# zprodev/zlib.es

Measured on AMD Instinct MI355X. Metric: GiB/s deflate+inflate round trip, 64 MiB buffers (uncompressed bytes / wall), bit-exact vs reference, higher is better.
Workload: dtype u8; 1 GPU; random64: 1 x 64 MiB xorshift buffer(s) per GPU (seed 12345+index), deflate then inflate, HBM-resident; bytes_per_buffer=67108864, compressed_bytes=67176156, parallelism=independent buffers, one per GPU

## Files before the change

zlib.es_amd/csrc/zes_deflate.hip:

```cpp
#include "zes_common.h"
#include "zes_kernels.h"

__device__ static inline uint32_t lds_ld32u(const uint8_t* s, uint32_t off) {
  const uint32_t* w = reinterpret_cast<const uint32_t*>(s);
  uint32_t i = off >> 2;
  uint32_t lo = w[i], hi = w[i + 1];
  return __builtin_amdgcn_alignbyte(hi, lo, off & 3u);
}

__device__ static inline void stage_block(uint8_t* s, const uint8_t* g, uint32_t bytes, uint32_t padded) {
  const uint32_t tid = threadIdx.x, nth = blockDim.x;
  const uint32_t mis = (uint32_t)((uintptr_t)g & 15u);
  if (mis == 0) {
    const uint4* g4 = reinterpret_cast<const uint4*>(g);
    uint4* s4 = reinterpret_cast<uint4*>(s);
    const uint32_t full = bytes >> 4;
    for (uint32_t i = tid; i < full; i += nth) s4[i] = g4[i];
    for (uint32_t i = (full << 4) + tid; i < padded; i += nth) s[i] = i < bytes ? g[i] : (uint8_t)0;
  } else {
    for (uint32_t i = tid; i < padded; i += nth) s[i] = i < bytes ? g[i] : (uint8_t)0;
  }
}

__device__ unsigned long long* g_sort_dbg = nullptr;
// ... 2191 lines not shown
      if ((int)lane >= d) incl += t;
    }
    if (lane == 63) S.wsum[wave] = incl;
    __syncthreads();
    uint32_t base = 14u + 3u * HCLEN, total = 0;
    for (uint32_t w = 0; w < HUFF_THREADS / 64; w++) {
      if (w < wave) base += S.wsum[w];
      total += S.wsum[w];
    }
    uint32_t bp = base + incl - mine;
    if (tb[0]) hdr_or(S, bp, tv[0], tb[0]);
    bp += tb[0];
    if (tb[1]) hdr_or(S, bp, tv[1], tb[1]);
    if (tid == 0) S.hdr_bits = 14u + 3u * HCLEN + total;
  }
  __syncthreads();
  USTAMP(6);
  uint32_t part = 0;
  for (uint32_t s = tid; s < 286; s += HUFF_THREADS) {
    uint32_t xb = (s >= 257) ? kLenXbits[s - 257] : 0u;
    part += hg[s] * ((uint32_t)S.lens[s] + xb);
  }
  if (tid < 30) part += hg[288 + tid] * ((uint32_t)S.lens[288 + tid] + kDistXbits[tid]);
  atomicAdd(&S.total_bits, part);
  __syncthreads();
  if (tid == 0) {
    blks[g].hdr_bits = S.hdr_bits;
    blks[g].bits = 3u + S.hdr_bits + S.total_bits;
  }
  uint32_t* cg = codes_out + (uint64_t)g * 320;
  for (uint32_t i = tid; i < 320; i += HUFF_THREADS) cg[i] = (uint32_t)S.codes[i] | ((uint32_t)S.lens[i] << 16);
  uint32_t* hd = hdr_out + (uint64_t)g * ZES_HDR_WORDS;
  for (uint32_t i = tid; i < ZES_HDR_WORDS; i += HUFF_THREADS) hd[i] = S.hdr[i];
  USTAMP(7);
}

__global__ __launch_bounds__(HUFF_THREADS) void k_huff_lengths_only(const uint32_t* __restrict__ hist, uint32_t nsym, uint32_t L,
                                                                    uint8_t* __restrict__ lens_out) {
  __shared__ HuffSmem S;
  const uint32_t tid = threadIdx.x;
  for (uint32_t i = tid; i < 320; i += HUFF_THREADS) S.hist[i] = i < nsym ? hist[i] : 0u;
  __syncthreads();
  pm_lengths(S, S.hist, nsym, L, S.lens);
  for (uint32_t i = tid; i < nsym; i += HUFF_THREADS) lens_out[i] = S.lens[i];
}

__global__ void k_make_blks(ZesBuf b0, uint32_t nbuf, ZesBuf* __restrict__ bufs, ZesBlk* __restrict__ blks, uint32_t nblk,
                            unsigned long long* __restrict__ adler) {
  const uint32_t i = blockIdx.x * blockDim.x + threadIdx.x;
  if (nbuf == 1u && i == 0) bufs[0] = b0;
  if (i < 2u * nbuf) adler[i] = 0ull;
  if (i >= nblk) return;
  uint32_t lo = 0, hi = nbuf;
  while (hi - lo > 1) {
    const uint32_t mid = (lo + hi) >> 1;
    if ((nbuf == 1u ? b0.first_blk : bufs[mid].first_blk) <= i) lo = mid; else hi = mid;
  }
  const uint64_t n = nbuf == 1u ? b0.n : bufs[lo].n;
  const uint32_t fb = nbuf == 1u ? b0.first_blk : bufs[lo].first_blk;
  ZesBlk z;
  z.buf = lo;
  z.blk = i - fb;
  z.len = (uint32_t)min((uint64_t)ZES_BLK, n - (uint64_t)z.blk * ZES_BLK);
  z.ntok = 0;
  z.hdr_bits = 0;
  z.bits = 0;
  z.bit_off = 0;
  blks[i] = z;
}

__device__ __forceinline__ static void adler_group_sums(uint4 v, uint32_t& a, uint32_t& w) {
  a = __builtin_amdgcn_udot4(v.x, 0x01010101u, 0u, false);
  a = __builtin_amdgcn_udot4(v.y, 0x01010101u, a, false);
  a = __builtin_amdgcn_udot4(v.z, 0x01010101u, a, false);
  a = __builtin_amdgcn_udot4(v.w, 0x01010101u, a, false);
  w = __builtin_amdgcn_udot4(v.x, 0x0D0E0F10u, 0u, false);
  w = __builtin_amdgcn_udot4(v.y, 0x090A0B0Cu, w, false);
  w = __builtin_amdgcn_udot4(v.z, 0x05060708u, w, false);
  w = __builtin_amdgcn_udot4(v.w, 0x01020304u, w, false);
}

__device__ __forceinline__ static void adler_chunk(const uint8_t* __restrict__ p0, uint64_t n, uint64_t c0, uint64_t clen,
                                                   unsigned long long* __restrict__ acc) {
  __shared__ uint64_t sa[ADLER_THREADS / 64], sb[ADLER_THREADS / 64];
  const uint32_t tid = threadIdx.x, lane = tid & 63u, wave = tid >> 6;
  const uint8_t* p = p0 + c0;
  uint64_t A = 0, B = 0;
  const bool aligned = (((uintptr_t)p) & 15u) == 0;
  uint64_t o_first = (uint64_t)tid * 16;
  if (aligned) {
    constexpr uint64_t ROUND = (uint64_t)ADLER_THREADS * 16 * 4;
    const uint64_t nround = clen / ROUND;
    for (uint64_t r = 0; r < nround; r++) {
      uint4 v[4];
#pragma unroll
      for (uint32_t q = 0; q < 4; q++) v[q] = *reinterpret_cast<const uint4*>(p + r * ROUND + (uint64_t)q * ADLER_THREADS * 16 + (uint64_t)tid * 16);
#pragma unroll
      for (uint32_t q = 0; q < 4; q++) {
        const uint64_t o = r * ROUND + (uint64_t)q * ADLER_THREADS * 16 + (uint64_t)tid * 16;
        uint32_t a, w;
        adler_group_sums(v[q], a, w);
        A += a;
        B += (uint64_t)w + (uint64_t)a * (clen - o - 16);
      }
    }
    o_first += nround * ROUND;
  }
  for (uint64_t o = o_first; o < clen; o += (uint64_t)ADLER_THREADS * 16) {
    uint8_t b[16];
    if (aligned && o + 16 <= clen) {
      *reinterpret_cast<uint4*>(b) = *reinterpret_cast<const uint4*>(p + o);
    } else {
#pragma unroll
      for (int k = 0; k < 16; k++) b[k] = (o + k < clen) ? p[o + k] : (uint8_t)0;
    }
    uint32_t a = 0, w = 0;
#pragma unroll
    for (int k = 0; k < 16; k++) {
      a += b[k];
      w += (uint32_t)(16 - k) * b[k];
    }
    A += a;
    B += (uint64_t)w + (uint64_t)a * (clen - o - 16);
  }
  for (int d = 32; d >= 1; d >>= 1) {
    A += __shfl_down(A, d);
    B += __shfl_down(B, d);
  }
  if (lane == 0) {
    sa[wave] = A;
    sb[wave] = B;
  }
  __syncthreads();
  if (tid == 0) {
    uint64_t ta = 0, tb = 0;
    for (uint32_t w = 0; w < ADLER_THREADS / 64; w++) {
      ta += sa[w];
      tb += sb[w];
    }
    const uint64_t after = n - c0 - clen;
    ta %= 65521u;
    tb %= 65521u;
    const uint64_t share = (tb + ta * (after % 65521u)) % 65521u;
    atomicAdd(&acc[0], (unsigned long long)ta);
    atomicAdd(&acc[1], (unsigned long long)share);
  }
}

__global__ __launch_bounds__(ADLER_THREADS) void k_adler(const uint8_t* __restrict__ d_in, uint64_t in_off, uint64_t n,
                                                         unsigned long long* __restrict__ acc) {
  const uint64_t c0 = (uint64_t)blockIdx.x * ADLER_CHUNK;
  adler_chunk(d_in + in_off, n, c0, min((uint64_t)ADLER_CHUNK, n - c0), acc);
}

__global__ __launch_bounds__(ADLER_THREADS) void k_adler_blocks(const uint8_t* __restrict__ d_in, const ZesBuf* __restrict__ bufs,
                                                                const ZesBlk* __restrict__ blks,
                                                                unsigned long long* __restrict__ acc) {
  const ZesBlk bk = blks[blockIdx.x];
  const ZesBuf bf = bufs[bk.buf];
  adler_chunk(d_in + bf.in_off, bf.n, (uint64_t)bk.blk * ZES_BLK, bk.len, acc + 2 * (size_t)bk.buf);
}

__device__ __forceinline__ static uint4 adler_low_bytes(uint32_t n) {
  const uint64_t lo = n >= 8u ? ~0ull : (1ull << (8u * n)) - 1ull;
  const uint64_t hi = n <= 8u ? 0ull : (n >= 16u ? ~0ull : (1ull << (8u * (n - 8u))) - 1ull);
  return make_uint4((uint32_t)lo, (uint32_t)(lo >> 32), (uint32_t)hi, (uint32_t)(hi >> 32));
}

__device__ __forceinline__ static void adler_seg_group(uint4 v, uint32_t o, uint32_t keep_lo, uint32_t keep_hi, uint64_t behind, uint64_t& A,
                                                       uint64_t& B) {
  if (o < keep_lo || o + 16u > keep_hi) {
    const uint4 ml = adler_low_bytes(keep_lo > o ? keep_lo - o : 0u);
    const uint4 mh = adler_low_bytes(keep_hi > o ? min(keep_hi - o, 16u) : 0u);
    v.x &= mh.x & ~ml.x;
    v.y &= mh.y & ~ml.y;
    v.z &= mh.z & ~ml.z;
    v.w &= mh.w & ~ml.w;
  }
  uint32_t a, w;
  adler_group_sums(v, a, w);
  A += a;
  B += (uint64_t)w + (uint64_t)a * behind;
}

__global__ __launch_bounds__(ADLER_THREADS) void k_adler_seg(const uint8_t* __restrict__ d_in, const ZesCrcSeg* __restrict__ segs,
                                                             const uint2* __restrict__ work, unsigned long long* __restrict__ acc) {
  __shared__ uint64_t sa[ADLER_THREADS / 64], sb[ADLER_THREADS / 64];
  const uint32_t tid = threadIdx.x, lane = tid & 63u, wave = tid >> 6;
  const uint2 wk = work[blockIdx.x];
  const ZesCrcSeg sg = segs[wk.x];
  const uint64_t a = (uint64_t)(uintptr_t)d_in + sg.off, end = a + sg.len;
  const uint64_t lo = (a & ~15ull) + (uint64_t)wk.y * ADLER_CHUNK;
  const uint64_t hi = min(lo + ADLER_CHUNK, (end + 15ull) & ~15ull);
  const uint32_t span = (uint32_t)(hi - lo);
  const uint32_t keep_lo = a > lo ? (uint32_t)(a - lo) : 0u;
  const uint32_t keep_hi = (uint32_t)(min(end, hi) - lo);
  const uint4* __restrict__ p = reinterpret_cast<const uint4*>((uintptr_t)lo);
  uint64_t A = 0, B = 0;
  constexpr uint32_t ROUND = ADLER_THREADS * 16u * 4u;
  const uint32_t nround = span / ROUND;
  for (uint32_t r = 0; r < nround; r++) {
    uint4 v[4];
#pragma unroll
    for (uint32_t q = 0; q < 4; q++) v[q] = p[(r * ROUND + q * ADLER_THREADS * 16u) / 16u + tid];
#pragma unroll
    for (uint32_t q = 0; q < 4; q++) {
      const uint32_t o = r * ROUND + q * ADLER_THREADS * 16u + tid * 16u;
      adler_seg_group(v[q], o, keep_lo, keep_hi, (uint64_t)keep_hi - o - 16u, A, B);
    }
  }
  for (uint32_t o = nround * ROUND + tid * 16u; o < span; o += ADLER_THREADS * 16u)
    adler_seg_group(p[o / 16u], o, keep_lo, keep_hi, (uint64_t)keep_hi - o - 16u, A, B);
  for (int d = 32; d >= 1; d >>= 1) {
    A += __shfl_down(A, d);
    B += __shfl_down(B, d);
  }
  if (lane == 0) {
    sa[wave] = A;
    sb[wave] = B;
  }
  __syncthreads();
  if (tid == 0) {
    uint64_t ta = 0, tb = 0;
    for (uint32_t w = 0; w < ADLER_THREADS / 64; w++) {
      ta += sa[w];
      tb += sb[w];
    }
    const uint64_t after = end - min(end, hi);
    ta %= 65521u;
    tb %= 65521u;
    const uint64_t share = (tb + ta * (after % 65521u)) % 65521u;
    atomicAdd(&acc[2 * (size_t)wk.x], (unsigned long long)ta);
    atomicAdd(&acc[2 * (size_t)wk.x + 1], (unsigned long long)share);
  }
}

__global__ __launch_bounds__(256) void k_layout(uint8_t* __restrict__ d_out, const ZesBuf* __restrict__ bufs,
                                                ZesBlk* __restrict__ blks, const unsigned long long* __restrict__ adler_acc,
                                                ZesRes* __restrict__ res) {
  __shared__ uint64_t s_tot;
  __shared__ uint64_t s_part[256];
  const uint32_t b = blockIdx.x, tid = threadIdx.x;
  const ZesBuf bf = bufs[b];
  ZesBlk* bk = blks + bf.first_blk;
  uint32_t* out32 = reinterpret_cast<uint32_t*>(d_out + bf.out_off);
  {
    const uint32_t per = (bf.nblk + 255u) / 256u;
    const uint32_t lo = min(bf.nblk, tid * per), hi = min(bf.nblk, lo + per);
    uint64_t sum = 0;
    for (uint32_t i = lo; i < hi; i++) sum += bk[i].bits;
    s_part[tid] = sum;
    __syncthreads();
    if (tid == 0) {
      uint64_t off = (bf.flags & ZES_BUF_RANGE) ? bf.start_bit : 16;
      for (uint32_t t = 0; t < 256; t++) {
        const uint64_t v = s_part[t];
        s_part[t] = off;
        off += v;
      }
      s_tot = off;
    }
    __syncthreads();
    uint64_t off = s_part[tid];
    for (uint32_t i = lo; i < hi; i++) {
      bk[i].bit_off = off;
      off += bk[i].bits;
    }
  }
  __syncthreads();
  const uint64_t tot = s_tot;
  const bool range = (bf.flags & ZES_BUF_RANGE) != 0;
  const uint64_t raw_end = (tot + 7) >> 3;
  const uint64_t out_len = raw_end + (range ? 0 : 4);
  for (uint32_t i = tid; i < bf.nblk; i += 256) {
    const uint64_t s = bk[i].bit_off, e = s + bk[i].bits - 1;
    if (!(i == 0 && (bf.flags & ZES_BUF_CONT) && (s & 31u))) out32[s >> 5] = 0;
    out32[e >> 5] = 0;
  }
  __syncthreads();
  if (tid == 0) {
    const uint64_t last_dw = (tot - 1) >> 5;
    const uint64_t end_dw = (out_len * 8 - 1) >> 5;
    for (uint64_t w = last_dw + 1; w <= end_dw; w++) out32[w] = 0;
    __threadfence();
    const uint64_t n = bf.n;
    const uint32_t s1 = (uint32_t)((1ull + adler_acc[2 * b + 0]) % 65521ull);
    const uint32_t s2 = (uint32_t)((n % 65521ull + adler_acc[2 * b + 1]) % 65521ull);
    const uint32_t ad = (s2 << 16) | s1;
    if (!range) {
      atomicOr(&out32[0], 0x9C78u);
      for (int k = 0; k < 4; k++) {
        const uint64_t pos = raw_end + k;
        const uint32_t byte = (ad >> (24 - 8 * k)) & 0xffu;
        atomicOr(&out32[pos >> 2], byte << (8 * (pos & 3)));
      }
    }
    res[b].out_len = range ? tot - bf.start_bit : out_len;
    res[b].status = 0;
    res[b].aux = ad;
  }
}

#ifndef EMIT_ITEMS
#define EMIT_ITEMS 4
#endif
#define EMIT_TILE (EMIT_THREADS * EMIT_ITEMS)
#define EMIT_STAGE_WORDS (EMIT_TILE * 48 / 32 + 8)
struct EmitSmem {
  uint32_t codes[320];
  uint32_t stage[EMIT_STAGE_WORDS];
  uint32_t wsum[EMIT_THREADS / 64];
  uint32_t carry;
};

__device__ static inline void stage_or(uint32_t* stage, uint32_t rel_bit, uint64_t v, uint32_t nbits) {
  const uint32_t w = rel_bit >> 5, sh = rel_bit & 31u;
  const uint64_t lo = v << sh;
  atomicOr(&stage[w], (uint32_t)lo);
  if (sh + nbits > 32u) atomicOr(&stage[w + 1], (uint32_t)(lo >> 32));
  if (sh + nbits > 64u) atomicOr(&stage[w + 2], (uint32_t)(v >> (64u - sh)));
}

__device__ __forceinline__ static void emit_lds_barrier() { asm volatile("s_waitcnt lgkmcnt(0)\n\ts_barrier" ::: "memory"); }

__global__ __launch_bounds__(EMIT_THREADS, 8) void k_emit(uint8_t* __restrict__ d_out, const ZesBuf* __restrict__ bufs,
                                                       const ZesBlk* __restrict__ blks, const uint32_t* __restrict__ tok_in,
                                                       const uint32_t* __restrict__ codes_in, const uint32_t* __restrict__ hdr_in) {
  __shared__ EmitSmem S;
  const uint32_t g = blockIdx.x, tid = threadIdx.x, lane = tid & 63u, wave = tid >> 6;
  const ZesBlk bk = blks[g];
  const ZesBuf bf = bufs[bk.buf];
  uint32_t* out32 = reinterpret_cast<uint32_t*>(d_out + bf.out_off);
  const uint32_t* tk = tok_in + (uint64_t)g * ZES_BLK;
  const uint32_t* hd = hdr_in + (uint64_t)g * ZES_HDR_WORDS;
  for (uint32_t i = tid; i < 320; i += EMIT_THREADS) S.codes[i] = codes_in[(uint64_t)g * 320 + i];
  if (tid == 0) S.carry = 0;
  const uint64_t blk_first_dw = bk.bit_off >> 5;
  const uint64_t blk_last_dw = (bk.bit_off + bk.bits - 1) >> 5;
  const bool is_final = (bk.blk + 1 == bf.nblk) && !(bf.flags & ZES_BUF_NOTFINAL);
  const uint32_t nhdr_items = 1 + ((bk.hdr_bits + 31u) >> 5);
  const uint32_t nitems = EMIT_TILE + bk.ntok + 1;
  static_assert(1 + ZES_HDR_WORDS <= EMIT_TILE, "header items fit the first tile");
  uint64_t cur_bit = bk.bit_off;
  __syncthreads();

  uint4 pre[EMIT_ITEMS / 4];
#pragma unroll
  for (int k4 = 0; k4 < EMIT_ITEMS / 4; k4++) pre[k4] = make_uint4(0, 0, 0, 0);
  for (uint32_t t0 = 0; t0 < nitems; t0 += EMIT_TILE) {
    uint64_t val[EMIT_ITEMS];
    uint32_t nb[EMIT_ITEMS];
    uint32_t mysum = 0;
    uint32_t tv4[EMIT_ITEMS];
#pragma unroll
    for (int k4 = 0; k4 < EMIT_ITEMS / 4; k4++) {
      tv4[4 * k4 + 0] = pre[k4].x;
      tv4[4 * k4 + 1] = pre[k4].y;
      tv4[4 * k4 + 2] = pre[k4].z;
      tv4[4 * k4 + 3] = pre[k4].w;
    }
    {
      const uint32_t ti0 = t0 + tid * EMIT_ITEMS;
      const uint4* qp = reinterpret_cast<const uint4*>(tk + min(ti0, ZES_BLK - EMIT_ITEMS));
#pragma unroll
      for (int k4 = 0; k4 < EMIT_ITEMS / 4; k4++) pre[k4] = qp[k4];
    }
#pragma unroll
    for (int k = 0; k < EMIT_ITEMS; k++) {
      const uint32_t it = t0 + tid * EMIT_ITEMS + k;
      uint64_t v = 0;
      uint32_t b = 0;
      if (it < EMIT_TILE) {
        if (it == 0) {
          v = (is_final ? 1u : 0u) | (2u << 1);
          b = 3;
        } else if (it < nhdr_items) {
          const uint32_t wi = it - 1;
          v = hd[wi];
          b = min(32u, bk.hdr_bits - wi * 32u);
        }
      } else if (it < nitems) {
        if (it == nitems - 1) {
          const uint32_t c = S.codes[256];
          v = c & 0xffffu;
          b = c >> 16;
        } else {
          const uint32_t tv = tv4[k];
          if (tv & ZES_TOK_MATCH) {
            const uint32_t len = zes_tok_len(tv), dist = zes_tok_dist(tv);
            const uint32_t lc = zes_len_code(len), dc = zes_dist_code(dist);
            const uint32_t cl = S.codes[257 + lc], cd = S.codes[288 + dc];
            const uint32_t ll = cl >> 16, dl = cd >> 16;
            const uint32_t lx = kLenXbits[lc], dx = kDistXbits[dc];
            v = (uint64_t)(cl & 0xffffu);
            b = ll;
            v |= (uint64_t)(len - kLenBase[lc]) << b;
            b += lx;
            v |= (uint64_t)(cd & 0xffffu) << b;
            b += dl;
            v |= (uint64_t)(dist - kDistBase[dc]) << b;
            b += dx;
          } else {
            const uint32_t c = S.codes[tv];
            v = c & 0xffffu;
            b = c >> 16;
          }
        }
      }
      val[k] = v;
      nb[k] = b;
      mysum += b;
    }
    uint32_t incl = mysum;
#pragma unroll
    for (int d = 1; d < 64; d <<= 1) {
      const uint32_t t = __shfl_up(incl, d);
      if ((int)lane >= d) incl += t;
    }
    if (lane == 63) S.wsum[wave] = incl;
    emit_lds_barrier();
    uint32_t wbase = 0, tile_bits = 0;
#pragma unroll
    for (uint32_t w = 0; w < EMIT_THREADS / 64; w++) {
      const uint32_t s = S.wsum[w];
      if (w < wave) wbase += s;
      tile_bits += s;
    }
    uint32_t rel = wbase + incl - mysum;
    const uint32_t head = (uint32_t)(cur_bit & 31u);
    const uint32_t nwords = (head + tile_bits + 31u) >> 5;
    for (uint32_t i = tid; i < nwords + 1; i += EMIT_THREADS) S.stage[i] = (i == 0) ? S.carry : 0u;
    emit_lds_barrier();
    rel += head;
    {
      uint64_t acc = 0;
      uint32_t accn = 0, accpos = rel;
#pragma unroll
      for (int k = 0; k < EMIT_ITEMS; k++) {
        if (accn + nb[k] > 64u) {
          stage_or(S.stage, accpos, acc, accn);
          accpos += accn;
          acc = 0;
          accn = 0;
        }
        acc |= val[k] << accn;
        accn += nb[k];
      }
      if (accn) stage_or(S.stage, accpos, acc, accn);
    }
    emit_lds_barrier();
    const uint64_t first_dw = cur_bit >> 5;
    const uint32_t end_bits = head + tile_bits;
    const bool last_tile = (t0 + EMIT_TILE >= nitems);
    const uint32_t ncomplete = last_tile ? nwords : (end_bits >> 5);
    for (uint32_t i = tid; i < ncomplete; i += EMIT_THREADS) {
      const uint64_t gw = first_dw + i;
      const uint32_t w = S.stage[i];
      if (gw == blk_first_dw || gw == blk_last_dw) atomicOr(&out32[gw], w);
      else out32[gw] = w;
    }
    const uint32_t carry_next = (!last_tile && (end_bits & 31u)) ? S.stage[end_bits >> 5] : 0u;
    emit_lds_barrier();
    if (tid == 0) S.carry = carry_next;
    cur_bit += tile_bits;
  }
}

__global__ __launch_bounds__(256) void k_bits_place(uint32_t* __restrict__ dst, uint64_t pos, const uint32_t* __restrict__ src, uint64_t nbits) {
  if (!nbits) return;
  const uint64_t first = pos >> 5, last = (pos + nbits - 1) >> 5;
  const uint32_t sh = (uint32_t)(pos & 31u);
  const uint64_t nsrc = (nbits + 31) >> 5;
  for (uint64_t w = first + (uint64_t)blockIdx.x * blockDim.x + threadIdx.x; w <= last; w += (uint64_t)gridDim.x * blockDim.x) {
    const uint64_t k = w - first;
    uint32_t lo = 0, hi = 0;
    if (k < nsrc) hi = src[k];
    if (k >= 1 && k - 1 < nsrc) lo = src[k - 1];
    uint32_t v = sh ? ((hi << sh) | (lo >> (32u - sh))) : hi;
    const uint64_t bit_lo = w << 5;
    if (bit_lo + 32 > pos + nbits) v &= (uint32_t)((1ull << (pos + nbits - bit_lo)) - 1ull);
    if (bit_lo < pos) v &= ~(uint32_t)((1ull << (pos - bit_lo)) - 1ull);
    if (w == first || w == last) atomicOr(&dst[w], v);
    else dst[w] = v;
  }
}

__global__ __launch_bounds__(SORT_THREADS) void k_selftest_lds_order(unsigned long long* __restrict__ out, uint32_t iters, uint32_t seed) {
  __shared__ uint32_t row[SORT_WAVES][128];
  const uint32_t tid = threadIdx.x, lane = tid & 63u, wave = tid >> 6;
  unsigned long long bad = 0, n = 0;
  for (uint32_t it = 0; it < iters; it++) {
    row[wave][lane] = 0;
    row[wave][lane + 64u] = 0;
    const uint32_t pat = (it + wave) % 6u;
    uint32_t h = seed ^ (blockIdx.x * 0x9E3779B1u) ^ (it * SORT_THREADS + tid);
    h = (h ^ (h >> 16)) * 0x7feb352du;
    h = (h ^ (h >> 15)) * 0x846ca68bu;
    h ^= h >> 16;
    uint32_t d;
    if (pat == 0) d = h & 255u;
    else if (pat == 1) d = h & 3u;
    else if (pat == 2) d = 77u + (lane >> 6);
    else if (pat == 3) d = 32u + ((h >> 3) % 27u);
    else if (pat == 4) d = (h & 1u) + 2u * ((h >> 8) & 7u);
    else d = (lane * 4u + (h & 3u)) & 255u;
    const bool valid = pat != 3u || (h >> 20) % 9u != 0u;
    uint32_t dd[4], rk[4];
#pragma unroll
    for (int r = 0; r < 4; r++) dd[r] = (d + (pat == 0u ? 17u * r : 0u)) & 255u;
#pragma unroll
    for (int r = 0; r < 4; r++) {
      const uint32_t sh = 16u * (dd[r] & 1u);
      const uint32_t old = valid ? atomicAdd(&row[wave][dd[r] >> 1], 1u << sh) : 0u;
      rk[r] = (old >> sh) & 0xffffu;
    }
#pragma unroll
    for (int r = 0; r < 4; r++) {
      uint32_t expect = 0;
      for (int q = 0; q <= r; q++) {
        uint64_t m = __ballot(valid);
        for (int b = 0; b < 8; b++) {
          const bool bit = (dd[r] >> b) & 1u;
          const uint64_t bal = __ballot((dd[q] >> b) & 1u);
          m &= bit ? bal : ~bal;
        }
        expect += (uint32_t)__popcll(q < r ? m : (m & zes_lanemask_lt()));
      }
      if (valid) {
        n++;
        bad += rk[r] != expect;
      }
    }
  }
  atomicAdd(&out[0], bad);
  atomicAdd(&out[1], n);
}

__global__ void k_zero_u64(unsigned long long* p, uint32_t n) {
  const uint32_t i = blockIdx.x * blockDim.x + threadIdx.x;
  if (i < n) p[i] = 0ull;
}
```

Baseline: 45.63 GiB/s.

## Add 16-items-per-thread emit path with windowed staging for literal-heavy blocks

Adds a second k_emit variant that handles 16 tokens per thread when a block is mostly literals (ntok > len/2). It uses DPP wave scans, a bounded LDS window processed in rounds over waves, and direct stores instead of atomics for non-shared words. The intent is to cut per-tile barrier and atomic overhead in the emit stage for incompressible data, which is what the random input produces. The cost is more registers and LDS, which may lower occupancy, plus a branch at kernel entry that chooses between the two paths.

After: 45.54 GiB/s (median of 2 runs). About the same (-0.2%).

```diff
diff --git a/zlib.es_amd/csrc/zes_deflate.hip b/zlib.es_amd/csrc/zes_deflate.hip
--- a/zlib.es_amd/csrc/zes_deflate.hip
+++ b/zlib.es_amd/csrc/zes_deflate.hip
@@ -2517,18 +2517,244 @@
 }
 
 #ifndef EMIT_ITEMS
-#define EMIT_ITEMS 4
+#define EMIT_ITEMS 16
 #endif
 #define EMIT_TILE (EMIT_THREADS * EMIT_ITEMS)
-#define EMIT_STAGE_WORDS (EMIT_TILE * 48 / 32 + 8)
+#define EMIT_WAVES (EMIT_THREADS / 64)
+#define EMIT_WIN_WORDS (EMIT_TILE * 15 / 32 + ZES_HDR_WORDS + 8)
+#define EMIT_WIN_BITS ((EMIT_WIN_WORDS - 4) * 32u)
+static_assert(31u + 3u + ZES_HDR_WORDS * 32u + 64u * EMIT_ITEMS * 48u <= EMIT_WIN_BITS, "a single wave's tokens always fit a round");
+static_assert(EMIT_ITEMS % 4 == 0 && EMIT_TILE <= ZES_BLK, "16-byte token loads");
+static_assert(EMIT_WAVES == 16, "k_emit reads the waves' sums as four 16-byte words");
 struct EmitSmem {
+  uint32_t codes[324];
+  __attribute__((aligned(16))) uint32_t stage[EMIT_WIN_WORDS];
+  __attribute__((aligned(16))) uint32_t wsum[EMIT_WAVES];
+};
+
+__device__ static inline void stage_or(uint32_t* stage, uint32_t rel_bit, uint32_t v, uint32_t nbits) {
+  const uint32_t w = rel_bit >> 5, sh = rel_bit & 31u;
+  const uint64_t lo = (uint64_t)v << sh;
+  atomicOr(&stage[w], (uint32_t)lo);
+  if (sh + nbits > 32u) atomicOr(&stage[w + 1], (uint32_t)(lo >> 32));
+}
+
+__device__ __forceinline__ static void emit_lds_barrier() { asm volatile("s_waitcnt lgkmcnt(0)\n\ts_barrier" ::: "memory"); }
+
+template <int CTRL, int ROWS>
+__device__ __forceinline__ static uint32_t emit_dpp(uint32_t x) {
+  return (uint32_t)__builtin_amdgcn_update_dpp(0, (int)x, CTRL, ROWS, 0xf, false);
+}
+__device__ __forceinline__ static uint32_t emit_wave_scan(uint32_t x) {
+  x += emit_dpp<0x111, 0xf>(x);
+  x += emit_dpp<0x112, 0xf>(x);
+  x += emit_dpp<0x114, 0xf>(x);
+  x += emit_dpp<0x118, 0xf>(x);
+  x += emit_dpp<0x142, 0xa>(x);
+  x += emit_dpp<0x143, 0xc>(x);
+  return x;
+}
+__device__ __forceinline__ static uint32_t emit_uniform(uint32_t x) { return (uint32_t)__builtin_amdgcn_readfirstlane((int)x); }
+
+struct EmitMatch {
+  uint32_t v1, n1, v2, n2;
+};
+__device__ __forceinline__ static EmitMatch emit_match(const uint32_t* codes, uint32_t tv) {
+  asm volatile("" : "+v"(tv));
+  const uint32_t y = zes_tok_len(tv) - 3u, x = zes_tok_dist(tv) - 1u;
+  const uint32_t lc = zes_len_code(y + 3u), dc = zes_dist_code(x + 1u);
+  const uint32_t cl = codes[257u + lc], cd = codes[288u + dc];
+  const uint32_t ll = cl >> 16, dl = cd >> 16;
+  const uint32_t lx = (lc < 8u || lc == 28u) ? 0u : (lc - 4u) >> 2;
+  const uint32_t dx = dc < 4u ? 0u : (dc >> 1) - 1u;
+  EmitMatch m;
+  m.v1 = (cl & 0xffffu) | ((y & ((1u << lx) - 1u)) << ll);
+  m.n1 = ll + lx;
+  m.v2 = (cd & 0xffffu) | ((x & ((1u << dx) - 1u)) << dl);
+  m.n2 = dl + dx;
+  return m;
+}
+
+__device__ __forceinline__ static void emit_block_by16(uint8_t* __restrict__ d_out, const ZesBuf* __restrict__ bufs,
+                                                       const ZesBlk* __restrict__ blks, const uint32_t* __restrict__ tok_in,
+                                                       const uint32_t* __restrict__ codes_in, const uint32_t* __restrict__ hdr_in) {
+  __shared__ EmitSmem S;
+  const uint32_t g = blockIdx.x, tid = threadIdx.x, lane = tid & 63u, wave = emit_uniform(tid >> 6);
+  const ZesBlk bk = blks[g];
+  const ZesBuf bf = bufs[bk.buf];
+  uint32_t* out32 = reinterpret_cast<uint32_t*>(d_out + bf.out_off);
+  const uint32_t* tk = tok_in + (uint64_t)g * ZES_BLK;
+  const uint32_t* hd = hdr_in + (uint64_t)g * ZES_HDR_WORDS;
+  uint4 pre[EMIT_ITEMS / 4];
+  {
+    const uint4* qp = reinterpret_cast<const uint4*>(tk + min(tid * EMIT_ITEMS, ZES_BLK - EMIT_ITEMS));
+#pragma unroll
+    for (int k4 = 0; k4 < EMIT_ITEMS / 4; k4++) pre[k4] = qp[k4];
+  }
+  for (uint32_t i = tid; i < 320; i += EMIT_THREADS) S.codes[i] = codes_in[(uint64_t)g * 320 + i];
+  if (tid == 0) S.codes[320] = 0;
+  const uint64_t blk_first_dw = bk.bit_off >> 5;
+  const uint64_t blk_last_dw = (bk.bit_off + bk.bits - 1) >> 5;
+  const bool is_final = (bk.blk + 1 == bf.nblk) && !(bf.flags & ZES_BUF_NOTFINAL);
+  const uint32_t nhdr_items = 1 + ((bk.hdr_bits + 31u) >> 5);
+  static_assert(1 + ZES_HDR_WORDS <= EMIT_THREADS, "a header item per thread");
+  const uint32_t ntok = bk.ntok;
+  uint64_t win_dw = blk_first_dw;
+  uint32_t head = (uint32_t)(bk.bit_off & 31u) + 3u + bk.hdr_bits;
+  uint32_t zfrom = ((head >> 5) + 4u) & ~3u;
+  uint32_t carry = 0;
+  for (uint32_t i = tid; i < zfrom; i += EMIT_THREADS) S.stage[i] = 0;
+  __syncthreads();
+  if (tid < nhdr_items) {
+    const uint32_t wi = tid - 1u;
+    const uint32_t v = tid == 0 ? ((is_final ? 1u : 0u) | (2u << 1)) : hd[wi];
+    const uint32_t b = tid == 0 ? 3u : min(32u, bk.hdr_bits - wi * 32u);
+    stage_or(S.stage, (uint32_t)(bk.bit_off & 31u) + (tid == 0 ? 0u : 3u + wi * 32u), v, b);
+  }
+
+  for (uint32_t t0 = 0; t0 <= ntok; t0 += EMIT_TILE) {
+    uint32_t tv[EMIT_ITEMS];
+#pragma unroll
+    for (int k4 = 0; k4 < EMIT_ITEMS / 4; k4++) {
+      tv[4 * k4 + 0] = pre[k4].x;
+      tv[4 * k4 + 1] = pre[k4].y;
+      tv[4 * k4 + 2] = pre[k4].z;
+      tv[4 * k4 + 3] = pre[k4].w;
+    }
+    uint32_t tq = threadIdx.x;
+    asm volatile("" : "+v"(tq));
+    tq *= EMIT_ITEMS;
+    {
+      const uint32_t ti0 = t0 + EMIT_TILE + tq;
+      const uint4* qp = reinterpret_cast<const uint4*>(tk + min(ti0, ZES_BLK - EMIT_ITEMS));
+#pragma unroll
+      for (int k4 = 0; k4 < EMIT_ITEMS / 4; k4++) pre[k4] = qp[k4];
+    }
+    const uint32_t it0 = t0 + tq;
+    if (it0 + EMIT_ITEMS > ntok) {
+#pragma unroll
+      for (int k = 0; k < EMIT_ITEMS; k++) {
+        const uint32_t it = it0 + (uint32_t)k;
+        if (it >= ntok) tv[k] = it == ntok ? 256u : 320u;
+      }
+    }
+    uint32_t mysum = 0;
+#pragma unroll
+    for (int k = 0; k < EMIT_ITEMS; k++) {
+      const uint32_t t = tv[k];
+      if (t & ZES_TOK_MATCH) {
+        const EmitMatch m = emit_match(S.codes, t);
+        mysum += m.n1 + m.n2;
+      } else {
+        const uint32_t c = S.codes[t];
+        tv[k] = c;
+        mysum += c >> 16;
+      }
+    }
+    const uint32_t incl = emit_wave_scan(mysum);
+    if (lane == 63) S.wsum[wave] = incl;
+    emit_lds_barrier();
+    const bool last_tile = t0 + EMIT_TILE > ntok;
+    uint32_t wb = 0, pb = 0;
+    for (;;) {
+      uint32_t we = wb + 1u, pe = pb, wbase = 0;
+      {
+        const uint4* w4 = reinterpret_cast<const uint4*>(S.wsum);
+        uint32_t run = 0, wv = wave;
+        asm volatile("" : "+s"(wv));
+#pragma unroll
+        for (uint32_t q = 0; q < EMIT_WAVES / 4; q++) {
+          const uint4 v = w4[q];
+          const uint32_t s4[4] = {emit_uniform(v.x), emit_uniform(v.y), emit_uniform(v.z), emit_uniform(v.w)};
+#pragma unroll
+          for (uint32_t j = 0; j < 4; j++) {
+            const uint32_t w = 4u * q + j;
+            wbase = (w == wv) ? run : wbase;
+            run += s4[j];
+            if (w >= wb && head + (run - pb) <= EMIT_WIN_BITS) {
+              we = w + 1u;
+              pe = run;
+            }
+          }
+        }
+      }
+      const uint32_t end_bits = head + (pe - pb);
+      const uint32_t nwords = (end_bits + 31u) >> 5;
+      for (uint32_t i = zfrom + tid * 4u; i <= nwords; i += EMIT_THREADS * 4u)
+        *reinterpret_cast<uint4*>(&S.stage[i]) = make_uint4(i == 0 ? carry : 0u, 0u, 0u, 0u);
+      emit_lds_barrier();
+      if (wave >= wb && wave < we) {
+        const uint32_t rel = head + (wbase - pb) + (incl - mysum);
+        uint32_t w = rel >> 5, held = rel & 31u;
+        uint64_t acc = 0;
+        bool shared = held != 0;
+        auto add = [&](uint32_t v, uint32_t n) {
+          acc |= (uint64_t)v << held;
+          held += n;
+        };
+        auto flush = [&]() {
+          if (held >= 32u) {
+            if (shared) atomicOr(&S.stage[w], (uint32_t)acc);
+            else S.stage[w] = (uint32_t)acc;
+            shared = false;
+            w++;
+            acc >>= 32;
+            held -= 32u;
+          }
+        };
+#pragma unroll
+        for (int k = 0; k < EMIT_ITEMS; k++) {
+          uint32_t t = tv[k];
+          asm volatile("" : "+v"(t));
+          uint32_t v = t & 0xffffu, n = t >> 16;
+          const bool ism = (t & ZES_TOK_MATCH) != 0;
+          if (ism) {
+            const EmitMatch m = emit_match(S.codes, t);
+            flush();
+            add(m.v1, m.n1);
+            flush();
+            v = m.v2;
+            n = m.n2;
+          }
+          add(v, n);
+          if ((k & 1) || ism) flush();
+        }
+        if (mysum && held) atomicOr(&S.stage[w], (uint32_t)acc);
+      }
+      emit_lds_barrier();
+      const bool last = last_tile && we == EMIT_WAVES;
+      const uint32_t ncomplete = last ? nwords : (end_bits >> 5);
+      const uint64_t i_first = blk_first_dw - win_dw, i_last = blk_last_dw - win_dw;
+      const uint32_t a0 = i_first < ncomplete ? (uint32_t)i_first : ~0u, a1 = i_last < ncomplete ? (uint32_t)i_last : ~0u;
+      uint32_t* ow = out32 + win_dw;
+      for (uint32_t i = tid; i < ncomplete; i += EMIT_THREADS) {
+        const uint32_t w = S.stage[i];
+        if (i == a0 || i == a1) atomicOr(&ow[i], w);
+        else ow[i] = w;
+      }
+      carry = (!last && (end_bits & 31u)) ? emit_uniform(S.stage[end_bits >> 5]) : 0u;
+      win_dw += end_bits >> 5;
+      head = end_bits & 31u;
+      zfrom = 0;
+      if (we == EMIT_WAVES) break;
+      wb = we;
+      pb = pe;
+      emit_lds_barrier();
+    }
+  }
+}
+
+#define EMIT4_ITEMS 4
+#define EMIT4_TILE (EMIT_THREADS * EMIT4_ITEMS)
+#define EMIT4_STAGE_WORDS (EMIT4_TILE * 48 / 32 + 8)
+struct Emit4Smem {
   uint32_t codes[320];
-  uint32_t stage[EMIT_STAGE_WORDS];
+  uint32_t stage[EMIT4_STAGE_WORDS];
   uint32_t wsum[EMIT_THREADS / 64];
   uint32_t carry;
 };
 
-__device__ static inline void stage_or(uint32_t* stage, uint32_t rel_bit, uint64_t v, uint32_t nbits) {
+__device__ static inline void stage_or64(uint32_t* stage, uint32_t rel_bit, uint64_t v, uint32_t nbits) {
   const uint32_t w = rel_bit >> 5, sh = rel_bit & 31u;
   const uint64_t lo = v << sh;
   atomicOr(&stage[w], (uint32_t)lo);
@@ -2536,12 +2762,10 @@
   if (sh + nbits > 64u) atomicOr(&stage[w + 2], (uint32_t)(v >> (64u - sh)));
 }
 
-__device__ __forceinline__ static void emit_lds_barrier() { asm volatile("s_waitcnt lgkmcnt(0)\n\ts_barrier" ::: "memory"); }
-
-__global__ __launch_bounds__(EMIT_THREADS, 8) void k_emit(uint8_t* __restrict__ d_out, const ZesBuf* __restrict__ bufs,
-                                                       const ZesBlk* __restrict__ blks, const uint32_t* __restrict__ tok_in,
-                                                       const uint32_t* __restrict__ codes_in, const uint32_t* __restrict__ hdr_in) {
-  __shared__ EmitSmem S;
+__device__ __forceinline__ static void emit_block_by4(uint8_t* __restrict__ d_out, const ZesBuf* __restrict__ bufs, const ZesBlk* __restrict__ blks,
+                                                       const uint32_t* __restrict__ tok_in, const uint32_t* __restrict__ codes_in,
+                                                       const uint32_t* __restrict__ hdr_in) {
+  __shared__ Emit4Smem S;
   const uint32_t g = blockIdx.x, tid = threadIdx.x, lane = tid & 63u, wave = tid >> 6;
   const ZesBlk bk = blks[g];
   const ZesBuf bf = bufs[bk.buf];
@@ -2554,38 +2778,38 @@
   const uint64_t blk_last_dw = (bk.bit_off + bk.bits - 1) >> 5;
   const bool is_final = (bk.blk + 1 == bf.nblk) && !(bf.flags & ZES_BUF_NOTFINAL);
   const uint32_t nhdr_items = 1 + ((bk.hdr_bits + 31u) >> 5);
-  const uint32_t nitems = EMIT_TILE + bk.ntok + 1;
-  static_assert(1 + ZES_HDR_WORDS <= EMIT_TILE, "header items fit the first tile");
+  const uint32_t nitems = EMIT4_TILE + bk.ntok + 1;
+  static_assert(1 + ZES_HDR_WORDS <= EMIT4_TILE, "header items fit the first tile");
   uint64_t cur_bit = bk.bit_off;
   __syncthreads();
 
-  uint4 pre[EMIT_ITEMS / 4];
-#pragma unroll
-  for (int k4 = 0; k4 < EMIT_ITEMS / 4; k4++) pre[k4] = make_uint4(0, 0, 0, 0);
-  for (uint32_t t0 = 0; t0 < nitems; t0 += EMIT_TILE) {
-    uint64_t val[EMIT_ITEMS];
-    uint32_t nb[EMIT_ITEMS];
+  uint4 pre[EMIT4_ITEMS / 4];
+#pragma unroll
+  for (int k4 = 0; k4 < EMIT4_ITEMS / 4; k4++) pre[k4] = make_uint4(0, 0, 0, 0);
+  for (uint32_t t0 = 0; t0 < nitems; t0 += EMIT4_TILE) {
+    uint64_t val[EMIT4_ITEMS];
+    uint32_t nb[EMIT4_ITEMS];
     uint32_t mysum = 0;
-    uint32_t tv4[EMIT_ITEMS];
-#pragma unroll
-    for (int k4 = 0; k4 < EMIT_ITEMS / 4; k4++) {
+    uint32_t tv4[EMIT4_ITEMS];
+#pragma unroll
+    for (int k4 = 0; k4 < EMIT4_ITEMS / 4; k4++) {
       tv4[4 * k4 + 0] = pre[k4].x;
       tv4[4 * k4 + 1] = pre[k4].y;
       tv4[4 * k4 + 2] = pre[k4].z;
       tv4[4 * k4 + 3] = pre[k4].w;
     }
     {
-      const uint32_t ti0 = t0 + tid * EMIT_ITEMS;
-      const uint4* qp = reinterpret_cast<const uint4*>(tk + min(ti0, ZES_BLK - EMIT_ITEMS));
-#pragma unroll
-      for (int k4 = 0; k4 < EMIT_ITEMS / 4; k4++) pre[k4] = qp[k4];
-    }
-#pragma unroll
-    for (int k = 0; k < EMIT_ITEMS; k++) {
-      const uint32_t it = t0 + tid * EMIT_ITEMS + k;
+      const uint32_t ti0 = t0 + tid * EMIT4_ITEMS;
+      const uint4* qp = reinterpret_cast<const uint4*>(tk + min(ti0, ZES_BLK - EMIT4_ITEMS));
+#pragma unroll
+      for (int k4 = 0; k4 < EMIT4_ITEMS / 4; k4++) pre[k4] = qp[k4];
+    }
+#pragma unroll
+    for (int k = 0; k < EMIT4_ITEMS; k++) {
+      const uint32_t it = t0 + tid * EMIT4_ITEMS + k;
       uint64_t v = 0;
       uint32_t b = 0;
-      if (it < EMIT_TILE) {
+      if (it < EMIT4_TILE) {
         if (it == 0) {
           v = (is_final ? 1u : 0u) | (2u << 1);
           b = 3;
@@ -2651,9 +2875,9 @@
       uint64_t acc = 0;
       uint32_t accn = 0, accpos = rel;
 #pragma unroll
-      for (int k = 0; k < EMIT_ITEMS; k++) {
+      for (int k = 0; k < EMIT4_ITEMS; k++) {
         if (accn + nb[k] > 64u) {
-          stage_or(S.stage, accpos, acc, accn);
+          stage_or64(S.stage, accpos, acc, accn);
           accpos += accn;
           acc = 0;
           accn = 0;
@@ -2661,12 +2885,12 @@
         acc |= val[k] << accn;
         accn += nb[k];
       }
-      if (accn) stage_or(S.stage, accpos, acc, accn);
+      if (accn) stage_or64(S.stage, accpos, acc, accn);
     }
     emit_lds_barrier();
     const uint64_t first_dw = cur_bit >> 5;
     const uint32_t end_bits = head + tile_bits;
-    const bool last_tile = (t0 + EMIT_TILE >= nitems);
+    const bool last_tile = (t0 + EMIT4_TILE >= nitems);
     const uint32_t ncomplete = last_tile ? nwords : (end_bits >> 5);
     for (uint32_t i = tid; i < ncomplete; i += EMIT_THREADS) {
       const uint64_t gw = first_dw + i;
@@ -2679,6 +2903,14 @@
     if (tid == 0) S.carry = carry_next;
     cur_bit += tile_bits;
   }
+}
+
+__global__ __launch_bounds__(EMIT_THREADS, 8) void k_emit(uint8_t* __restrict__ d_out, const ZesBuf* __restrict__ bufs,
+                                                       const ZesBlk* __restrict__ blks, const uint32_t* __restrict__ tok_in,
+                                                       const uint32_t* __restrict__ codes_in, const uint32_t* __restrict__ hdr_in) {
+  const ZesBlk bk = blks[blockIdx.x];
+  if (2u * bk.ntok > bk.len) emit_block_by16(d_out, bufs, blks, tok_in, codes_in, hdr_in);
+  else emit_block_by4(d_out, bufs, blks, tok_in, codes_in, hdr_in);
 }
 
 __global__ __launch_bounds__(256) void k_bits_place(uint32_t* __restrict__ dst, uint64_t pos, const uint32_t* __restrict__ src, uint64_t nbits) {
```
